# befelix/safe_learning

Measured on AMD Instinct MI355X. Metric: grid-cell Lyapunov checks/sec + ms/safe_set-update, 4D 128^4 grid, 1k-pt GP, higher is better.
Workload: dtype f64

## Files before the change

### include/sl_hip.h

```cpp
#ifndef SL_HIP_H
#define SL_HIP_H

#include <stdint.h>

#ifdef __cplusplus
extern "C" {
#endif

#define SL_API __attribute__((visibility("default")))

#define SL_OK               0
#define SL_ERR_INVALID     (-1)
#define SL_ERR_HIP         (-2)
#define SL_ERR_UNSUPPORTED (-3)
#define SL_ERR_NOMEM       (-4)

#define SL_MAX_STATE_DIM   6
#define SL_MAX_ACTION_DIM  2
#define SL_MAX_INPUT_DIM   8
#define SL_MAX_GP_HEADS    6
#define SL_MAX_NN_LAYERS   4
#define SL_MAX_SIMPLICES   32

typedef struct sl_ctx sl_ctx;
// ... 89 lines not shown
SL_API int  sl_version(void);
SL_API int  sl_ctx_create(int device, void* hip_stream, sl_ctx** out);
SL_API int  sl_ctx_destroy(sl_ctx* ctx);
SL_API const char* sl_last_error(const sl_ctx* ctx);
SL_API int  sl_ctx_synchronize(sl_ctx* ctx);
SL_API const char* sl_last_kernel(const sl_ctx* ctx);
SL_API int  sl_timing_configure(sl_ctx* ctx, int slots);
SL_API int  sl_timing_collect(sl_ctx* ctx, int channel, double* h_ms, int capacity, int* count);

SL_API int  sl_model_set(sl_ctx* ctx, const sl_model_desc* h_model);
SL_API int  sl_policy_touch(sl_ctx* ctx);

SL_API int  sl_gp_set_head(sl_ctx* ctx, int head, int n, int p, int dout, int col0,
                    const double* h_X, const double* h_Linv, const double* h_alpha,
                    double variance, const double* h_lengthscales);
#define SL_KERNEL_RBF 0
#define SL_KERNEL_MATERN32 1
#define SL_KERNEL_LINEAR 2
#define SL_KERNEL_MAX_FACTORS 8
typedef struct sl_gp_kernel_factor {
    int32_t kind, product;
    double  variance[SL_MAX_INPUT_DIM];
    double  inv_lengthscales[SL_MAX_INPUT_DIM];
} sl_gp_kernel_factor;
typedef struct sl_gp_kernel {
    int32_t nfactors, reserved;
    sl_gp_kernel_factor factor[SL_KERNEL_MAX_FACTORS];
} sl_gp_kernel;
SL_API int  sl_gp_set_head_kernel(sl_ctx* ctx, int head, int n, int p, int dout, int col0,
                    const double* h_X, const double* h_Linv, const double* h_alpha,
                    const sl_gp_kernel* h_kernel);
SL_API int  sl_gp_append_point(sl_ctx* ctx, int head, const double* h_x, const double* h_linv_row,
                        const double* h_alpha_new);
SL_API int  sl_gp_configure(sl_ctx* ctx, int nheads, double beta);
SL_API int  sl_gp4_early_configure(sl_ctx* ctx, int enable);
SL_API int  sl_gp4_workgroups_configure(sl_ctx* ctx, int workgroups);
SL_API int  sl_gp4_segment_configure(sl_ctx* ctx, int tiles);

SL_API int  sl_tri_set(sl_ctx* ctx, int slot, const sl_grid_desc* h_grid, int nsimplex,
                const int32_t* h_simplices, const double* h_hyperplanes,
                const double* h_discrete_points, int project, int ncols, const double* d_table);
SL_API int  sl_tri_set_table(sl_ctx* ctx, int slot, const double* d_table);

SL_API int  sl_network_set(sl_ctx* ctx, int nlayers, const int32_t* h_dims ,
                    const int32_t* h_activations, const double* h_kernels);

SL_API int  sl_policy_network_set(sl_ctx* ctx, int nlayers, const int32_t* h_dims,
                           const int32_t* h_activations, const double* h_kernels,
                           const double* h_biases, const int32_t* h_has_bias, double output_scale);

SL_API int  sl_values(sl_ctx* ctx, int64_t lo, int64_t hi, double* d_values);

SL_API int  sl_lyap_sweep(sl_ctx* ctx, int64_t lo, int64_t hi, const uint64_t* d_init_bits,
                   const double* d_values, uint64_t* d_neg_bits, sl_sweep_result* d_result,
                   double* d_dbg);


SL_API int  sl_values_implicit(sl_ctx* ctx, int* out);

SL_API int  sl_fold_results(sl_ctx* ctx, const sl_sweep_result* d_records, int count,
                     sl_sweep_result* d_out);

SL_API int  sl_lyap_finalize_dev(sl_ctx* ctx, int64_t lo, int64_t hi, const double* d_values,
                          const uint64_t* d_init_bits, const uint64_t* d_prev_bits,
                          const sl_sweep_result* d_folded, const sl_key* d_keep,
                          uint64_t* d_safe_bits, sl_sweep_result* d_result);
// ... 150 lines not shown
```

### safe_learning_amd/_hip.py

```python

import ctypes as C
import os

import numpy as np

HERE = os.path.dirname(os.path.abspath(__file__))
LIB_PATH = os.environ.get("SL_LIB_PATH") or os.path.join(HERE, "libslhip.so")

MAX_STATE_DIM = 6
MAX_ACTION_DIM = 2
MAX_INPUT_DIM = 8
MAX_GP_HEADS = 6
MAX_NN_LAYERS = 4
MAX_SIMPLICES = 32

OK, ERR_INVALID, ERR_HIP, ERR_UNSUPPORTED, ERR_NOMEM = 0, -1, -2, -3, -4
POLICY_LINEAR, POLICY_CONST, POLICY_TABLE, POLICY_TRI, POLICY_NETWORK = 1, 2, 3, 4, 5
DYN_LINEAR, DYN_PENDULUM, DYN_CARTPOLE, DYN_GP = 1, 2, 3, 4
V_QUADRATIC, V_TRI, V_NETWORK = 1, 2, 3
LIP_CONST, LIP_ABS_LINEAR, LIP_NORM_LINEAR, LIP_ABS_GRAD, LIP_NORM_GRAD = 0, 1, 2, 3, 4
LF_CONST, LF_AFFINE_NORM1 = 0, 1
EVAL_VALUE, EVAL_POLICY, EVAL_DYNAMICS, EVAL_DECREASE, EVAL_LV = 1, 2, 3, 4, 5
NN_LOSS_ABS, NN_LOSS_ROA = 1, 2

# ... 74 lines not shown
                ("jacobi_cycles", C.c_int64), ("residual_inf", C.c_double), ("bound", C.c_double),
                ("kappa", C.c_double), ("converged", C.c_int32), ("reserved", C.c_int32)]


SOLVE_GMRES, SOLVE_JACOBI = 0, 1


RESULT_WORDS = 8
R_FAIL_V, R_FAIL_I, R_LAST_V, R_LAST_I, R_MAX_V, R_MAX_I, R_BELOW, R_SAFE = range(8)
SORT_COUNT_WORDS = 256 * 2048
ADAPTIVE_ROW_WORDS = 6
SELECT_WORDS = 8
S_PREFIX, S_REMAINING, S_KEY_V, S_KEY_I, S_RANK, S_NONE = range(6)

_vp, _i64, _int, _dbl = C.c_void_p, C.c_int64, C.c_int, C.c_double
_int32_p = C.POINTER(C.c_int32)

SIGNATURES = {
    "sl_version": (_int, ()),
    "sl_ctx_create": (_int, (_int, _vp, C.POINTER(_vp))),
    "sl_ctx_destroy": (_int, (_vp,)),
    "sl_last_error": (C.c_char_p, (_vp,)),
    "sl_ctx_synchronize": (_int, (_vp,)),
    "sl_last_kernel": (C.c_char_p, (_vp,)),
    "sl_timing_configure": (_int, (_vp, _int)),
    "sl_timing_collect": (_int, (_vp, _int, c_double_p, _int, C.POINTER(_int))),
    "sl_model_set": (_int, (_vp, C.POINTER(ModelDesc))),
    "sl_policy_touch": (_int, (_vp,)),
    "sl_gp_set_head": (_int, (_vp, _int, _int, _int, _int, _int, c_double_p, c_double_p, c_double_p, _dbl,
                              c_double_p)),
    "sl_gp_set_head_kernel": (_int, (_vp, _int, _int, _int, _int, _int, c_double_p, c_double_p, c_double_p,
                                     C.POINTER(GpKernel))),
    "sl_gp_append_point": (_int, (_vp, _int, c_double_p, c_double_p, c_double_p)),
    "sl_gp_configure": (_int, (_vp, _int, _dbl)),
    "sl_gp4_early_configure": (_int, (_vp, _int)),
    "sl_gp4_workgroups_configure": (_int, (_vp, _int)),
    "sl_gp4_segment_configure": (_int, (_vp, _int)),
    "sl_tri_set": (_int, (_vp, _int, C.POINTER(GridDesc), _int, _int32_p, c_double_p, c_double_p, _int, _int,
                          _vp)),
    "sl_tri_set_table": (_int, (_vp, _int, _vp)),
    "sl_network_set": (_int, (_vp, _int, _int32_p, _int32_p, c_double_p)),
    "sl_policy_network_set": (_int, (_vp, _int, _int32_p, _int32_p, c_double_p, c_double_p, _int32_p, _dbl)),
    "sl_values": (_int, (_vp, _i64, _i64, _vp)),
    "sl_lyap_sweep": (_int, (_vp, _i64, _i64, _vp, _vp, _vp, _vp, _vp)),
    "sl_values_implicit": (_int, (_vp, C.POINTER(_int))),
    "sl_fold_results": (_int, (_vp, _vp, _int, _vp)),
    "sl_lyap_finalize_dev": (_int, (_vp, _i64, _i64, _vp, _vp, _vp, _vp, _vp, _vp, _vp)),
    "sl_refinement_carry": (_int, (_vp, _i64, _i64, _vp, _vp, _vp, _vp, _vp, _vp)),
    "sl_select_begin": (_int, (_vp, _vp, _i64, _i64, _vp, _i64)),
    "sl_select_hist": (_int, (_vp, _i64, _i64, _vp, _int, _int, _vp, _vp)),
    "sl_select_digit": (_int, (_vp, _int, _int, _vp, _vp)),
    "sl_sort_pairs": (_int, (_vp, _i64, _vp, _vp, _vp, _vp, _vp)),
    "sl_partition_by_digit": (_int, (_vp, _i64, _vp, _vp, _vp, _vp)),
    "sl_gather_rows": (_int, (_vp, _i64, _int, _vp, _vp, _vp)),
    "sl_adaptive_pack": (_int, (_vp, _i64, _i64, _vp, _vp, _int, _vp, _vp, _vp, _vp)),
    "sl_adaptive_dest": (_int, (_vp, _i64, _vp, _vp, _int, _vp)),
    "sl_adaptive_sort_keys": (_int, (_vp, _i64, _vp, _vp, _vp)),
    "sl_adaptive_analyse": (_int, (_vp, _i64, _i64, _i64, _vp, _vp, _dbl, _dbl, _i64, _vp, _vp)),
    "sl_adaptive_apply": (_int, (_vp, _i64, _i64, _i64, _vp, _vp, _vp, _dbl, _dbl, _i64, _vp)),
    "sl_adaptive_scatter": (_int, (_vp, _i64, _i64, _i64, _vp, _vp, _vp, _vp, _vp)),
    "sl_index_to_state": (_int, (_vp, _i64, _vp, _vp)),
    "sl_perturb_pairs": (_int, (_vp, _i64, _int, _int, _vp, _vp, _int, _vp, _vp, _vp)),
    "sl_rows_sort_key": (_int, (_vp, _i64, _int, _int, _vp, _vp, _vp)),
    "sl_rows_duplicate_flags": (_int, (_vp, _i64, _int, _vp, _vp, _vp)),
    "sl_sample_bounds": (_int, (_vp, _i64, _int, _int, _vp, _vp, _vp, _dbl, _vp, _vp)),
    "sl_state_membership": (_int, (_vp, _i64, _vp, _vp, _vp)),
# ... 145 lines not shown
        alpha, pA = _as_c(alpha)
        ls, pls = _as_c(lengthscales)
        n, p = X.shape
        self.lib.sl_gp_set_head(self.handle, head, n, p, alpha.shape[1], col0, pX, pL, pA, float(variance),
                                pls)

    def gp_set_head_kernel(self, head, X, Linv, alpha, col0, factors):
        X, pX = _as_c(X)
        Linv, pL = _as_c(Linv)
        alpha, pA = _as_c(alpha)
        n, p = X.shape
        if len(factors) > KERNEL_MAX_FACTORS:
            raise ValueError("kernel with %d leaf factors (engine limit %d)" % (len(factors), KERNEL_MAX_FACTORS))
        spec = GpKernel()
        spec.nfactors = len(factors)
        for f, (kind, product, variance, inv_ls) in enumerate(factors):
            spec.factor[f].kind, spec.factor[f].product = int(kind), int(product)
            for q in range(p):
                spec.factor[f].variance[q] = float(variance[q])
                spec.factor[f].inv_lengthscales[q] = float(inv_ls[q])
        self.lib.sl_gp_set_head_kernel(self.handle, head, n, p, alpha.shape[1], col0, pX, pL, pA,
                                       C.byref(spec))

    def gp_append_point(self, head, x, linv_row, alpha_new):
        x, px = _as_c(x)
        row, pr = _as_c(linv_row)
        a, pa = _as_c(alpha_new)
        rc = self.lib.sl_gp_append_point(self.handle, head, px, pr, pa)
        if rc == ERR_UNSUPPORTED:
            return False
        self.check(rc, "sl_gp_append_point")
        return True

    def gp_inputs(self, head, n, p):
        out = np.empty((p, n), dtype=np.float64)
        self.lib.sl_debug_gp_inputs(self.handle, head, out.ctypes.data_as(c_double_p))
        return out

    def gp_configure(self, nheads, beta):
        self.lib.sl_gp_configure(self.handle, nheads, float(beta))

    def tri_set(self, slot, grid_desc, simplices, hyperplanes, discrete_points, project, ncols,
                table):
        simplices = np.ascontiguousarray(simplices, dtype=np.int32)
        hyper, ph = _as_c(hyperplanes)
        pts, pp = _as_c(np.concatenate(discrete_points))
        self._keepalive[slot] = table
        self.lib.sl_tri_set(self.handle, slot, C.byref(grid_desc), len(simplices),
                            simplices.ctypes.data_as(C.POINTER(C.c_int32)), ph, pp, int(bool(project)),
                            ncols, _ptr(table))

    def tri_set_table(self, slot, table):
        self._keepalive[slot] = table
        self.lib.sl_tri_set_table(self.handle, slot, _ptr(table))

    def network_set(self, dims, activations, kernels):
        dims = np.ascontiguousarray(dims, dtype=np.int32)
        acts = np.ascontiguousarray(activations, dtype=np.int32)
        flat, pk = _as_c(np.concatenate([np.asarray(k, dtype=np.float64).ravel() for k in kernels]))
        self.lib.sl_network_set(self.handle, len(acts), dims.ctypes.data_as(C.POINTER(C.c_int32)),
                                acts.ctypes.data_as(C.POINTER(C.c_int32)), pk)

    def policy_network_set(self, dims, activations, kernels, biases, output_scale):
        dims = np.ascontiguousarray(dims, dtype=np.int32)
        acts = np.ascontiguousarray(activations, dtype=np.int32)
        flat, pk = _as_c(np.concatenate([np.asarray(k, dtype=np.float64).ravel() for k in kernels]))
# ... 278 lines not shown
```

### safe_learning_amd/csrc/sl_gp.hip

```cpp
#include "sl_common.h"

typedef double sl_d4 __attribute__((ext_vector_type(4)));
typedef double sl_d2 __attribute__((ext_vector_type(2)));

#define SL_GP_SLABS_PER_CHUNK 16
#ifndef SL_GP_STAGGER
#define SL_GP_STAGGER 1
#endif
#ifndef SL_GP_GEN_UNROLL
#define SL_GP_GEN_UNROLL 1
#endif
#define SL_GP_DOUT_MAX SL_MAX_STATE_DIM

static constexpr int kCfgW[2] = {4, 8};
static constexpr int kCfgR[2] = {1, 4};
static constexpr int kCfgCB[2] = {1, 4};

static inline int cfg_panel_rows(int cfg) { return 16 * kCfgR[cfg != 0] * kCfgW[cfg != 0]; }

template <int W, int R, int CB, bool GENERAL, int DT, int MT, bool XSG = false>
__global__ __launch_bounds__(W * 64) void k_gp_sweep(
    const SlDevModel M, const SlGpDev gp, SlAux aux_arg, int64_t lo, int64_t hi, int64_t ntiles,
    const uint64_t* __restrict__ init_bits, const double* __restrict__ values,
    uint64_t* __restrict__ neg_bits, sl_key* __restrict__ partials, double* __restrict__ dbg,
    int xs_doubles, int alpha_doubles, const double* __restrict__ points, int nb_arg) {
    __shared__ SlTriLds<GENERAL> tri_lds;
    const SlAux aux = sl_stage_aux<GENERAL>(tri_lds, aux_arg);
    constexpr int C = 16 * CB;
    constexpr int RP = 16 * R * W;
    constexpr int RB = R * W;
    constexpr int FRAGS = SL_GP_SLABS_PER_CHUNK * CB / W;
    constexpr int KXBUF = SL_GP_SLABS_PER_CHUNK * CB * 64;
    static_assert(W % CB == 0, "W must be a multiple of CB");
// ... 283 lines not shown
    }
    __syncthreads();
    sl_block_reduce_key<true>(best_v, best_i, sv, si);
    if (tid == 0) { partials[blockIdx.x].vbits = best_v; partials[blockIdx.x].index = best_i; }
}

static int choose_cfg(const sl_ctx* ctx, int n) {
    if (ctx->env.gp_cfg >= 0) return ctx->env.gp_cfg;
    if (n <= 256) return 0;
    return 2;
}

static int gp_set_head(sl_ctx* ctx, int head, int n, int p, int dout, int col0, const double* h_X,
                       const double* h_Linv, const double* h_alpha, double variance,
                       const double* h_lengthscales, const sl_gp_kernel* h_kernel) {
    if (!ctx || !h_X || !h_Linv || !h_alpha || !h_lengthscales)
        return sl_fail(ctx, SL_ERR_INVALID, "sl_gp_set_head: NULL argument");
    if (head < 0 || head >= SL_MAX_GP_HEADS)
        return sl_fail(ctx, SL_ERR_INVALID, "sl_gp_set_head: head %d outside [0,%d)", head,
                       SL_MAX_GP_HEADS);
    if (n < 1 || p < 1 || p > SL_MAX_INPUT_DIM || dout < 1 || col0 < 0 ||
        col0 + dout > SL_MAX_STATE_DIM)
        return sl_fail(ctx, SL_ERR_INVALID, "sl_gp_set_head: bad sizes n=%d p=%d dout=%d col0=%d",
                       n, p, dout, col0);
    if (!(variance > 0.0)) return sl_fail(ctx, SL_ERR_INVALID, "sl_gp_set_head: variance <= 0");
    for (int q = 0; q < p; ++q)
        if (!(h_lengthscales[q] > 0.0))
            return sl_fail(ctx, SL_ERR_INVALID, "sl_gp_set_head: lengthscale <= 0");
    const int cfg = choose_cfg(ctx, n);
    const int rp = cfg_panel_rows(cfg);
    const int n_pad = ((n + rp - 1) / rp) * rp;
    const int nslab2 = n_pad / 8;

    std::vector<double> xs((size_t)p * n_pad, 0.0), alphap((size_t)n_pad * dout, 0.0);
    std::vector<double> mpack((size_t)n_pad * n_pad, 0.0);
    for (int j = 0; j < n; ++j)
        for (int q = 0; q < p; ++q) xs[(size_t)q * n_pad + j] = h_X[(size_t)j * p + q] / h_lengthscales[q];
    for (int i = 0; i < n; ++i) {
        for (int dd = 0; dd < dout; ++dd) {
            const double ai = h_alpha[(size_t)i * dout + dd];
            if (ai == 0.0) continue;
            for (int j = 0; j <= i; ++j) alphap[(size_t)j * dout + dd] += h_Linv[(size_t)i * n + j] * ai;
        }
    }
    for (int I = 0; I < n_pad / 16; ++I) {
        for (int S2 = 0; S2 < nslab2; ++S2) {
            if (8 * S2 > 16 * I + 15) continue;
            for (int l = 0; l < 64; ++l) {
                const int row = 16 * I + (l & 15);
                for (int e = 0; e < 2; ++e) {
                    const int col = 4 * (2 * S2 + e) + (l >> 4);
                    double v = 0.0;
                    if (row < n && col <= row) v = h_Linv[(size_t)row * n + col];
                    mpack[(((size_t)I * nslab2 + S2) * 64 + l) * 2 + e] = v;
                }
            }
        }
    }
    SL_HIP_CHECK(ctx, hipSetDevice(ctx->device));
    SL_HIP_CHECK(ctx, hipStreamSynchronize(ctx->stream));
    ++ctx->dynamics_token;
    SlGpHeadHost& hh = ctx->gp_heads[head];
    if (hh.d_xs) (void)hipFree(hh.d_xs);
    if (hh.d_mpack) (void)hipFree(hh.d_mpack);
    if (hh.d_alpha) (void)hipFree(hh.d_alpha);
    if (hh.d_kernel) (void)hipFree(hh.d_kernel);
    hh.d_xs = hh.d_mpack = hh.d_alpha = nullptr;
    hh.d_kernel = nullptr;
    if (h_kernel) {
        SL_HIP_CHECK(ctx, hipMalloc(&hh.d_kernel, sizeof(sl_gp_kernel)));
        SL_HIP_CHECK(ctx, hipMemcpy(hh.d_kernel, h_kernel, sizeof(sl_gp_kernel), hipMemcpyHostToDevice));
        hh.h_kernel = *h_kernel;
    }
    SL_HIP_CHECK(ctx, hipMalloc(&hh.d_xs, xs.size() * sizeof(double)));
    SL_HIP_CHECK(ctx, hipMalloc(&hh.d_mpack, mpack.size() * sizeof(double)));
    SL_HIP_CHECK(ctx, hipMalloc(&hh.d_alpha, alphap.size() * sizeof(double)));
// ... 67 lines not shown
    }
}

extern "C" int sl_gp_append_point(sl_ctx* ctx, int head, const double* h_x, const double* h_linv_row,
                                  const double* h_alpha_new) {
    if (!ctx || !h_x || !h_linv_row || !h_alpha_new)
        return sl_fail(ctx, SL_ERR_INVALID, "sl_gp_append_point: NULL argument");
    if (head < 0 || head >= SL_MAX_GP_HEADS || !ctx->gp_heads[head].set)
        return sl_fail(ctx, SL_ERR_INVALID, "sl_gp_append_point: head %d not set", head);
    SlGpHeadHost& hh = ctx->gp_heads[head];
    SlGpHeadDev& dv = ctx->h_gp.head[head];
    const int n = hh.n;
    if (n + 1 > hh.n_pad)
        return sl_fail(ctx, SL_ERR_UNSUPPORTED, "sl_gp_append_point: capacity %d of head %d is "
                                                "exhausted (upload the head again)", hh.n_pad, head);
    ++ctx->dynamics_token;
    SL_HIP_CHECK(ctx, hipSetDevice(ctx->device));
    SL_HIP_CHECK(ctx, hipStreamSynchronize(ctx->stream));
    const size_t need = sizeof(double) * (size_t)(n + 1 + hh.p + hh.dout);
    SL_HIP_CHECK(ctx, sl_grow(ctx, &ctx->d_scratch, &ctx->scratch_bytes, need));
    std::vector<double> stage((size_t)(n + 1 + hh.p + hh.dout));
    for (int c = 0; c <= n; ++c) stage[c] = h_linv_row[c];
    for (int q = 0; q < hh.p; ++q) stage[n + 1 + q] = h_x[q] / hh.lengthscales[q];
    for (int dd = 0; dd < hh.dout; ++dd) stage[n + 1 + hh.p + dd] = h_alpha_new[dd];
    double* d_stage = reinterpret_cast<double*>(ctx->d_scratch);
    SL_HIP_CHECK(ctx, hipMemcpy(d_stage, stage.data(), need, hipMemcpyHostToDevice));
    hipLaunchKernelGGL(k_gp_append, dim3((n + hh.p + 256) / 256), dim3(256), 0, ctx->stream, d_stage, n,
                       hh.n_pad, dv.nslab2, hh.p, hh.dout, d_stage + n + 1, d_stage + n + 1 + hh.p,
                       hh.d_mpack, hh.d_alpha, hh.d_xs);
    SL_HIP_CHECK(ctx, hipGetLastError());
    SL_HIP_CHECK(ctx, hipStreamSynchronize(ctx->stream));
    hh.n = n + 1;
    dv.n = n + 1;
    SL_HIP_CHECK(ctx, hipMemcpy(ctx->d_gp, &ctx->h_gp, sizeof(SlGpDev), hipMemcpyHostToDevice));
    return SL_OK;
}

extern "C" int sl_debug_gp_inputs(sl_ctx* ctx, int head, double* h_xs) {
    if (!ctx || !h_xs) return sl_fail(ctx, SL_ERR_INVALID, "sl_debug_gp_inputs: NULL argument");
    if (head < 0 || head >= SL_MAX_GP_HEADS || !ctx->gp_heads[head].set)
        return sl_fail(ctx, SL_ERR_INVALID, "sl_debug_gp_inputs: head %d not set", head);
    const SlGpHeadHost& hh = ctx->gp_heads[head];
    SL_HIP_CHECK(ctx, hipSetDevice(ctx->device));
    SL_HIP_CHECK(ctx, hipStreamSynchronize(ctx->stream));
    for (int q = 0; q < hh.p; ++q)
        SL_HIP_CHECK(ctx, hipMemcpy(h_xs + (size_t)q * hh.n, hh.d_xs + (size_t)q * hh.n_pad,
                                    sizeof(double) * hh.n, hipMemcpyDeviceToHost));
    return SL_OK;
}

extern "C" int sl_gp4_early_configure(sl_ctx* ctx, int enable) {
    if (!ctx) return sl_fail(nullptr, SL_ERR_INVALID, "sl_gp4_early_configure: NULL context");
    ctx->gp4_early = enable != 0;
    return SL_OK;
}

extern "C" int sl_gp_configure(sl_ctx* ctx, int nheads, double beta) {
    if (!ctx) return sl_fail(nullptr, SL_ERR_INVALID, "sl_gp_configure: NULL context");
    if (nheads < 1 || nheads > SL_MAX_GP_HEADS)
        return sl_fail(ctx, SL_ERR_INVALID, "sl_gp_configure: %d heads", nheads);
    int cfg = -1;
    for (int h = 0; h < nheads; ++h) {
        if (!ctx->gp_heads[h].set)
            return sl_fail(ctx, SL_ERR_INVALID, "sl_gp_configure: head %d not set", h);
        if (cfg < 0) cfg = ctx->gp_heads[h].cfg;
        if (cfg != ctx->gp_heads[h].cfg)
            return sl_fail(ctx, SL_ERR_UNSUPPORTED,
// ... 306 lines not shown
```

### safe_learning_amd/csrc/sl_gp4.hip

```cpp
#include "sl_common.h"
#include "sl_gp4_clobbers.h"
#include "sl_gp4_gen.h"
#include "sl_gp4_mean.h"
#include "sl_gp4_queue.h"

#ifdef SL_NO_GP4
bool sl_gp4_supports(const SlDevModel&) { return false; }
int sl_gp4_sweep_launch(sl_ctx* ctx, const SlDevModel&, const SlSweepArgs&, int*) {
    return sl_fail(ctx, SL_ERR_UNSUPPORTED, "k_gp_sweep4 is compiled out of this build");
}
extern "C" int sl_gp4_workgroups_configure(sl_ctx*, int) { return SL_OK; }
extern "C" int sl_gp4_segment_configure(sl_ctx*, int) { return SL_OK; }
#else

namespace gp4 {

#ifndef SL_GP4_R
#define SL_GP4_R 4
#endif
constexpr int R = SL_GP4_R, CB = 4, W = 4;
constexpr int NACC = R * CB * 4;
constexpr int C = 16 * CB;
constexpr int RP = 16 * R * W;
constexpr int RB = R * W;
#ifndef SL_GP4_WRITE_SKEW
#define SL_GP4_WRITE_SKEW 1
#endif
constexpr int KXS2 = CB * 128 + 4;
constexpr int KXBUF = 8 * KXS2;
static_assert(R == 4, "256-row panels (tools/audit_gp4.py is told the same number by the build)");

constexpr int REC_MEAN = 8, REC_SS = REC_MEAN + 16 * SL_D, REC = REC_SS + W * 16;
struct BlockCtl {
    Gp4Queues q;
    int action;
    int pos[GP4Q_SLOTS];
    int open[W];
    int push_stage;
    int src_done;
    int nsrc;
    int from_list;
    unsigned nlist;
};
constexpr int ACT_SOURCE = GP4Q_SOURCE, ACT_DONE = GP4Q_DONE;

struct AFrag { sl_d2 v[R]; };
struct BFrag { sl_d2 v[CB]; };

#define SL_A10(b) "a" #b "0", "a" #b "1", "a" #b "2", "a" #b "3", "a" #b "4", "a" #b "5", "a" #b "6", "a" #b "7", "a" #b "8", "a" #b "9"
#define SL_AGPRS_0_127                                                                             \
    "a0", "a1", "a2", "a3", "a4", "a5", "a6", "a7", "a8", "a9", SL_A10(1), SL_A10(2), SL_A10(3),   \
        SL_A10(4), SL_A10(5), SL_A10(6), SL_A10(7), SL_A10(8), SL_A10(9), SL_A10(10), SL_A10(11),   \
        "a120", "a121", "a122", "a123", "a124", "a125", "a126", "a127"
#define SL_ALL_AGPRS SL_AGPRS_0_127

template <int BASE>
__device__ __forceinline__ void acc_zero16() {
    asm volatile(
        "v_accvgpr_write_b32 a%c0, 0\n\tv_accvgpr_write_b32 a%c1, 0\n\tv_accvgpr_write_b32 a%c2, 0\n\t"
        "v_accvgpr_write_b32 a%c3, 0\n\tv_accvgpr_write_b32 a%c4, 0\n\tv_accvgpr_write_b32 a%c5, 0\n\t"
        "v_accvgpr_write_b32 a%c6, 0\n\tv_accvgpr_write_b32 a%c7, 0\n\tv_accvgpr_write_b32 a%c8, 0\n\t"
        "v_accvgpr_write_b32 a%c9, 0\n\tv_accvgpr_write_b32 a%c10, 0\n\tv_accvgpr_write_b32 a%c11, 0\n\t"
        "v_accvgpr_write_b32 a%c12, 0\n\tv_accvgpr_write_b32 a%c13, 0\n\tv_accvgpr_write_b32 a%c14, 0\n\t"
// ... 515 lines not shown
                const double* kxr = kx_l + buf * KXBUF + wave * 128 + own;
                sl_d2 kx[8];
                load_own_kx<KXS2>(kx, kxr);
                mean_mfma(kx, mi, macc);
            };
            auto produce = [&](int ch, int buf, int first_new, bool keep) {
                const bool with_mean = ch >= first_new && !(skip & 2);
                MeanIn mi;
                if (with_mean) load_alpha(mi, rs_alpha, lk, low, dout, ch);
                if (!(skip & 1)) generate(ch, buf, first_new, keep);
                if (with_mean) {
                    __builtin_amdgcn_fence(__ATOMIC_RELEASE, "wavefront");
                    __builtin_amdgcn_wave_barrier();
                    mean_run(buf, mi);
                }
            };

            const int npanels = (hd.n + RP - 1) / RP;
            constexpr int CPP = RP / 64;
            const int nchunks_head = npanels * CPP;
            auto decide_block = [&](int done) -> bool {
                const bool last = done == npanels;
                const int64_t idx = blk0 + lcol;
                const bool valid = lk == 0 && idx < hi;
                const int cl = 16 * wave + lcol;
                CellBounds b{false, false, 0.0};
                if (valid) {
                    double var = variance;
                    if (done > 0) {
                        double sumsq = 0.0;
                        for (int k = 0; k < PSS; ++k) sumsq += part_ss[k * C + cl];
                        var = variance - sumsq;
                    }
                    b = cell_bounds(M, nd, aux, gp.beta, idx, lo, points, values, cell_mean + cl * SL_D, var);
                }
                const bool neg_hi = b.neg_hi, open = b.open;
                const double v_x = b.v_x;
                const bool all = last || __ballot(open) == 0ull;
                if (all) {
                    const unsigned word = (unsigned)(__ballot(neg_hi) & 0xffffull);
                    const int64_t b16 = (blk0 - lo) >> 4;
                    unsigned init = 0u;
                    if (init_bits) init = reinterpret_cast<const unsigned short*>(init_bits)[b16];
                    if (lane == 0) reinterpret_cast<unsigned short*>(neg_bits)[b16] = (unsigned short)word;
                    const bool okc = neg_hi || ((init >> lcol) & 1u);
                    if (valid && !okc) sl_key_min(best_v, best_i, sl_vbits(v_x), idx);
#ifdef SL_DIAG
                    if (lane == 0 && !last && done < 4) atomicAdd(&sl_gp4_stage_count[done], 1ull);
#endif
                }
                return all;
            };
            if (early && stage == ACT_SOURCE) {
                for (int ch = 0; ch < nchunks_head; ++ch) produce(ch, ch & 1, 0, false);
                if (lk < dout)
                    cell_mean[(16 * wave + 4 * blk + low) * SL_D + hd.col0 + lk] = mean_sum(macc);
            }
#ifdef SL_DIAG
            if (early && stage >= 0 && stage < 4 && tid == 0) atomicAdd(&sl_gp4_stage_count[4 + stage], 1ull);
#endif
            for (int pan = early ? (stage >= 0 ? stage : npanels) : (decided ? npanels : 0);
                 pan < (early ? stage + 1 : npanels); ++pan) {
                acc_zero_all();
                int rowoff[R];
                int nzd[R];
#pragma unroll
                for (int r = 0; r < R; ++r) {
// ... 301 lines not shown
```

### safe_learning_amd/csrc/sl_gp4_gen.h

```cpp
#pragma once
#include "sl_common.h"

typedef double sl_d2 __attribute__((ext_vector_type(2)));
typedef unsigned sl_u4 __attribute__((ext_vector_type(4)));

namespace gp4 {

constexpr int RUNS = 4;
constexpr int RUNC = SL_P + 2;

__device__ __forceinline__ void exp_pair(double x1, double x2, double& e1, double& e2) {
    x1 = x1 < -800.0 ? -800.0 : x1;
    x2 = x2 < -800.0 ? -800.0 : x2;
    const double k1 = rint(x1 * 1.4426950408889634), k2 = rint(x2 * 1.4426950408889634);
    double r1 = fma(k1, -6.93147180369123816490e-01, x1), r2 = fma(k2, -6.93147180369123816490e-01, x2);
    r1 = fma(k1, -1.90821492927058770002e-10, r1);
    r2 = fma(k2, -1.90821492927058770002e-10, r2);
    double q1 = 1.6059043836821613e-10, q2 = 1.6059043836821613e-10;
#define SL_EXP_STEP(C) q1 = fma(q1, r1, C); q2 = fma(q2, r2, C)
    SL_EXP_STEP(2.08767569878681e-09);
    SL_EXP_STEP(2.505210838544172e-08);
    SL_EXP_STEP(2.755731922398589e-07);
    SL_EXP_STEP(2.7557319223985893e-06);
    SL_EXP_STEP(2.48015873015873e-05);
// ... 66 lines not shown
            rs_alpha, voff, (64 * ch + 8 * s2) * dout * 8, 0));
        mi.a1[s2] = __builtin_bit_cast(double, __builtin_amdgcn_raw_buffer_load_b64(
            rs_alpha, voff, (64 * ch + 8 * s2 + 4) * dout * 8, 0));
    }
}
template <int KXS2>
__device__ __forceinline__ void load_own_kx(sl_d2 (&kx)[8], const double* kxr) {
#pragma unroll
    for (int s2 = 0; s2 < 8; ++s2) kx[s2] = *reinterpret_cast<const sl_d2*>(kxr + s2 * KXS2);
}
__device__ __forceinline__ void mean_mfma(const sl_d2 (&kx)[8], const MeanIn& mi, double (&macc)[4]) {
#pragma unroll
    for (int h = 0; h < 2; ++h)
        asm volatile("s_nop 3\n\t"
                     "v_mfma_f64_4x4x4_4b_f64 %0, %4, %5, %0\n\t"
                     "v_mfma_f64_4x4x4_4b_f64 %1, %6, %7, %1\n\t"
                     "v_mfma_f64_4x4x4_4b_f64 %2, %8, %9, %2\n\t"
                     "v_mfma_f64_4x4x4_4b_f64 %3, %10, %11, %3\n\t"
                     "v_mfma_f64_4x4x4_4b_f64 %0, %12, %13, %0\n\t"
                     "v_mfma_f64_4x4x4_4b_f64 %1, %14, %15, %1\n\t"
                     "v_mfma_f64_4x4x4_4b_f64 %2, %16, %17, %2\n\t"
                     "v_mfma_f64_4x4x4_4b_f64 %3, %18, %19, %3"
                     : "+v"(macc[0]), "+v"(macc[1]), "+v"(macc[2]), "+v"(macc[3])
                     : "v"(mi.a0[4 * h]), "v"(kx[4 * h].x), "v"(mi.a1[4 * h]), "v"(kx[4 * h].y),
                       "v"(mi.a0[4 * h + 1]), "v"(kx[4 * h + 1].x), "v"(mi.a1[4 * h + 1]), "v"(kx[4 * h + 1].y),
                       "v"(mi.a0[4 * h + 2]), "v"(kx[4 * h + 2].x), "v"(mi.a1[4 * h + 2]), "v"(kx[4 * h + 2].y),
                       "v"(mi.a0[4 * h + 3]), "v"(kx[4 * h + 3].x), "v"(mi.a1[4 * h + 3]), "v"(kx[4 * h + 3].y));
    asm volatile("s_nop 15\n\ts_nop 7" : "+v"(macc[0]), "+v"(macc[1]), "+v"(macc[2]), "+v"(macc[3]));
}
__device__ __forceinline__ double mean_sum(const double (&macc)[4]) {
    return (macc[0] + macc[1]) + (macc[2] + macc[3]);
}

struct CellBounds { bool neg_hi, open; double v_x; };
__device__ __forceinline__ CellBounds cell_bounds(const SlDevModel& M, const SlDims& nd, const SlAux& aux, double beta,
                                                  int64_t idx, int64_t lo, const double* points, const double* values,
                                                  const double* mean_row, double var) {
    const int d = nd.d, p = nd.p;
    double x[SL_P], u[SL_M], prior[SL_D], mean[SL_D], err0[SL_D], err1[SL_D];
    sl_cell_state(M, d, idx, points, x);
    sl_policy_any<false>(M, nd, aux.tri, idx, x, u);
    sl_append_action(nd, u, x);
    sl_rows_dot<SL_D, SL_P>(M.m.dynamics.matrix, d, p, x, prior);
    const double e = beta * sqrt(var);
#pragma unroll
    for (int k = 0; k < SL_D; ++k) {
        if (k < d) {
            mean[k] = mean_row[k] + prior[k];
            err0[k] = 0.0;
            err1[k] = e;
        }
    }
    const SlCellCheck c0 = sl_cell_check<SL_FAST>(M, d, aux, x, mean, err0);
    const SlCellCheck c1 = sl_cell_check<SL_FAST>(M, d, aux, x, mean, err1);
    CellBounds b;
    b.neg_hi = c1.negative;
    b.open = c0.negative != c1.negative || !(fabs(c0.decrease) < INFINITY) || !(fabs(c1.decrease) < INFINITY);
    b.v_x = values ? values[idx - lo] : c1.v_x;
    return b;
}

}
```

### safe_learning_amd/csrc/sl_gp4_mean.hip

```cpp
#include "sl_common.h"
#include "sl_gp4_gen.h"
#include "sl_gp4_mean.h"
#include "sl_gp4_queue.h"

#ifndef SL_NO_GP4

namespace gp4m {

using gp4::RUNC;
using gp4::RUNS;
using gp4::uniform;

constexpr int W = 4;
constexpr int WG_PER_CU = 4;
constexpr int KXS2 = 128 + 4;
constexpr int KXBUF = 8 * KXS2;
constexpr int SLICE = KXBUF + 16 * SL_P + RUNS * RUNC;
static_assert(16 * SL_D <= KXBUF, "the block's means reuse the chunk buffer");
static_assert(W * SLICE * sizeof(double) <= 40 * 1024, "four workgroups of k_gp_mean_blocks per CU");

}

#ifdef SL_DIAG
static __device__ unsigned long long sl_gp4_mean_decided;
// ... 167 lines not shown
                        for (int c = c0; c < c1; ++c) {
                            kxw[2 * ((c + wswz) & 15)] = e;
                            e *= rho;
                            rho *= qr;
                        }
                    }
                } else {
                    gp4::direct_run(kxw, wswz, xv, cin, 0, variance, p);
                }
            };
            for (int ch = 0; ch < nchunks_head; ++ch) {
                const bool with_mean = !(skip & 2);
                gp4::MeanIn mi;
                if (with_mean) gp4::load_alpha(mi, rs_alpha, lk, low, dout, ch);
                if (!(skip & 1)) generate(ch);
                if (with_mean) {
                    __builtin_amdgcn_fence(__ATOMIC_RELEASE, "wavefront");
                    __builtin_amdgcn_wave_barrier();
                    sl_d2 kx[8];
                    gp4::load_own_kx<KXS2>(kx, kx_l + own);
                    gp4::mean_mfma(kx, mi, macc);
                }
            }
            __builtin_amdgcn_fence(__ATOMIC_RELEASE, "wavefront");
            __builtin_amdgcn_wave_barrier();
            if (lk < dout) cell_mean[(4 * blk + low) * SL_D + hd.col0 + lk] = gp4::mean_sum(macc);
            __builtin_amdgcn_fence(__ATOMIC_RELEASE, "wavefront");
            __builtin_amdgcn_wave_barrier();

            const int64_t idx = blk0 + lcol;
            const bool valid = lk == 0 && idx < hi;
            gp4::CellBounds b{false, false, 0.0};
            if (valid)
                b = gp4::cell_bounds(M, nd, aux, gp.beta, idx, lo, points, values, cell_mean + lcol * SL_D, variance);
            const bool neg_hi = b.neg_hi, open = b.open;
            const double v_x = b.v_x;
            if (__ballot(open) == 0ull) {
                const unsigned word = (unsigned)(__ballot(neg_hi) & 0xffffull);
                const int64_t b16 = (blk0 - lo) >> 4;
                unsigned init = 0u;
                if (init_bits) init = reinterpret_cast<const unsigned short*>(init_bits)[b16];
                if (lane == 0) reinterpret_cast<unsigned short*>(neg_bits)[b16] = (unsigned short)word;
                const bool okc = neg_hi || ((init >> lcol) & 1u);
                if (valid && !okc) sl_key_min(best_v, best_i, sl_vbits(v_x), idx);
#ifdef SL_DIAG
                if (lane == 0) atomicAdd(&sl_gp4_mean_decided, 1ull);
#endif
            } else {
                unsigned at = 0u;
                if (lane == 0) at = atomicAdd(list_count, 1u);
                at = (unsigned)__builtin_amdgcn_readfirstlane((int)at);
                if (at < list_cap) {
                    if (lane == 0) list_cell[at] = blk0;
                    double* rec = list_mean + (size_t)at * 16 * d;
                    for (int i = lane; i < 16 * d; i += 64) rec[i] = cell_mean[(i / d) * SL_D + i % d];
                }
            }
            __builtin_amdgcn_fence(__ATOMIC_RELEASE, "wavefront");
            __builtin_amdgcn_wave_barrier();
        }
    }
    sl_wave_reduce_key<true>(best_v, best_i);
    if (lane == 0) {
        sl_key* out = partials + blockIdx.x * W + wave;
        if (fold) sl_key_min(best_v, best_i, out->vbits, out->index);
        out->vbits = best_v;
        out->index = best_i;
// ... 56 lines not shown
```

### safe_learning_amd/csrc/sl_model.h

```cpp
#pragma once

#include <stdint.h>
#include <math.h>
#include <string.h>
#include "sl_hip.h"

#if defined(__HIPCC__)
#define SL_HD __host__ __device__ __forceinline__
#else
#define SL_HD inline
#endif

#define SL_D SL_MAX_STATE_DIM
#define SL_M SL_MAX_ACTION_DIM
#define SL_P SL_MAX_INPUT_DIM

#define SL_TRI_CODES   64
#define SL_TRI_MAXCAND 12
struct SlTri {
    sl_grid_desc grid;
    int32_t nsimplex, project, ncols, set;
    int32_t simplices[SL_MAX_SIMPLICES][SL_D + 1];
    double  hyper[SL_MAX_SIMPLICES][SL_D][SL_D];
    double  hyper_c[SL_MAX_SIMPLICES][SL_D];
// ... 827 lines not shown
SL_HD double sl_tanh(double x) {
#if defined(__HIP_DEVICE_COMPILE__)
    double y = -2.0 * fabs(x);
    y = y < -80.0 ? -80.0 : y;
    const double k = rint(y * 1.4426950408889634);
    double r = fma(k, -6.93147180369123816490e-01, y);
    r = fma(k, -1.90821492927058770002e-10, r);
    double q = 1.6059043836821613e-10;
    q = fma(q, r, 2.08767569878681e-09);
    q = fma(q, r, 2.505210838544172e-08);
    q = fma(q, r, 2.755731922398589e-07);
    q = fma(q, r, 2.7557319223985893e-06);
    q = fma(q, r, 2.48015873015873e-05);
    q = fma(q, r, 1.984126984126984e-04);
    q = fma(q, r, 1.3888888888888889e-03);
    q = fma(q, r, 8.333333333333333e-03);
    q = fma(q, r, 4.1666666666666664e-02);
    q = fma(q, r, 1.6666666666666666e-01);
    q = fma(q, r, 0.5);
    q = fma(q, r, 1.0);
    const double e = ldexp(fma(q, r, 1.0), (int)k);
    const double em1 = (k == 0.0) ? q * r : e - 1.0;
    const double t = (0.0 - em1) / (2.0 + em1);
    return copysign(t, x);
#else
    return tanh(x);
#endif
}
SL_HD double sl_act(int a, double x) { return a == 1 ? sl_tanh(x) : (a == 2 ? (x > 0.0 ? x : 0.0) : x); }
SL_HD double sl_dact(int a, double pre, double post) {
    return a == 1 ? (1.0 - post * post) : (a == 2 ? (pre > 0.0 ? 1.0 : 0.0) : 1.0);
}

struct SlGpHeadDev {
    int32_t n, n_pad, p, dout, col0, nslab2, reserved0, reserved1;
    double  variance;
    double  inv_ls[SL_P];
    const double* xs;
    const double* mpack;
    const double* alpha;
    const sl_gp_kernel* kernel;
};

SL_HD double sl_kernel_eval(const sl_gp_kernel& ks, int p, const double* a, const double* b) {
    double total = 0.0, prod = 1.0;
    int cur = 0;
    for (int f = 0; f < ks.nfactors; ++f) {
        const sl_gp_kernel_factor& fac = ks.factor[f];
        if (fac.product != cur) {
            total += prod;
            prod = 1.0;
            cur = fac.product;
        }
        double v = 0.0;
        if (fac.kind == SL_KERNEL_LINEAR) {
#pragma unroll
            for (int q = 0; q < SL_P; ++q)
                if (q < p) v = fma(a[q] * fac.variance[q], b[q], v);
        } else {
            double r2 = 0.0;
#pragma unroll
            for (int q = 0; q < SL_P; ++q) {
                if (q < p) {
                    const double dq = (a[q] - b[q]) * fac.inv_lengthscales[q];
                    r2 = fma(dq, dq, r2);
                }
// ... 370 lines not shown
```

Measured before the change: 272.1 million.

## Add certified GP variance lower bound to close cells earlier in staged gp4

```diff
diff --git a/include/sl_hip.h b/include/sl_hip.h
--- a/include/sl_hip.h
+++ b/include/sl_hip.h
@@ -145,6 +145,7 @@
                     const sl_gp_kernel* h_kernel);
 SL_API int  sl_gp_append_point(sl_ctx* ctx, int head, const double* h_x, const double* h_linv_row,
                         const double* h_alpha_new);
+SL_API int  sl_gp_variance_floor(sl_ctx* ctx, int head, double* out, int n);
 SL_API int  sl_gp_configure(sl_ctx* ctx, int nheads, double beta);
 SL_API int  sl_gp4_early_configure(sl_ctx* ctx, int enable);
 SL_API int  sl_gp4_workgroups_configure(sl_ctx* ctx, int workgroups);
diff --git a/safe_learning_amd/_hip.py b/safe_learning_amd/_hip.py
--- a/safe_learning_amd/_hip.py
+++ b/safe_learning_amd/_hip.py
@@ -130,6 +130,7 @@
     "sl_gp_set_head_kernel": (_int, (_vp, _int, _int, _int, _int, _int, c_double_p, c_double_p, c_double_p,
                                      C.POINTER(GpKernel))),
     "sl_gp_append_point": (_int, (_vp, _int, c_double_p, c_double_p, c_double_p)),
+    "sl_gp_variance_floor": (_int, (_vp, _int, c_double_p, _int)),
     "sl_gp_configure": (_int, (_vp, _int, _dbl)),
     "sl_gp4_early_configure": (_int, (_vp, _int)),
     "sl_gp4_workgroups_configure": (_int, (_vp, _int)),
@@ -341,6 +342,11 @@
         self.check(rc, "sl_gp_append_point")
         return True
 
+    def gp_variance_floor(self, head, stages):
+        out = np.zeros(stages, dtype=np.float64)
+        self.lib.sl_gp_variance_floor(self.handle, head, out.ctypes.data_as(c_double_p), stages)
+        return out
+
     def gp_inputs(self, head, n, p):
         out = np.empty((p, n), dtype=np.float64)
         self.lib.sl_debug_gp_inputs(self.handle, head, out.ctypes.data_as(c_double_p))
diff --git a/safe_learning_amd/csrc/sl_gp.hip b/safe_learning_amd/csrc/sl_gp.hip
--- a/safe_learning_amd/csrc/sl_gp.hip
+++ b/safe_learning_amd/csrc/sl_gp.hip
@@ -1,4 +1,5 @@
 #include "sl_common.h"
+#include "sl_gp_floor.h"
 
 typedef double sl_d4 __attribute__((ext_vector_type(4)));
 typedef double sl_d2 __attribute__((ext_vector_type(2)));
@@ -348,7 +349,7 @@
     const int n_pad = ((n + rp - 1) / rp) * rp;
     const int nslab2 = n_pad / 8;
 
-    std::vector<double> xs((size_t)p * n_pad, 0.0), alphap((size_t)n_pad * dout, 0.0);
+    std::vector<double> xs((size_t)p * n_pad, 0.0), alphap((size_t)n_pad * dout + SL_GP_FLOOR_WORDS, 0.0);
     std::vector<double> mpack((size_t)n_pad * n_pad, 0.0);
     for (int j = 0; j < n; ++j)
         for (int q = 0; q < p; ++q) xs[(size_t)q * n_pad + j] = h_X[(size_t)j * p + q] / h_lengthscales[q];
@@ -358,6 +359,14 @@
             if (ai == 0.0) continue;
             for (int j = 0; j <= i; ++j) alphap[(size_t)j * dout + dd] += h_Linv[(size_t)i * n + j] * ai;
         }
+    }
+    const int floor_stages = (n + SL_GP_FLOOR_RP - 1) / SL_GP_FLOOR_RP;
+    if (!h_kernel && ctx->gp4_early && ctx->env.gp_cfg < 0 && n_pad % SL_GP_FLOOR_RP == 0 &&
+        floor_stages <= SL_GP_FLOOR_STAGES && n <= SL_GP_FLOOR_MAX_N) {
+        double floor_c[SL_GP_FLOOR_STAGES] = {};
+        gpfloor::variance_floor(h_Linv, n, SL_GP_FLOOR_RP, floor_stages, variance, floor_c);
+        alphap[(size_t)n_pad * dout] = 2.0 * 64.0 * (double)n * 0x1p-53 * variance;
+        for (int s = 0; s < floor_stages; ++s) alphap[(size_t)n_pad * dout + 1 + s] = floor_c[s];
     }
     for (int I = 0; I < n_pad / 16; ++I) {
         for (int S2 = 0; S2 < nslab2; ++S2) {
@@ -491,7 +500,23 @@
     SL_HIP_CHECK(ctx, hipStreamSynchronize(ctx->stream));
     hh.n = n + 1;
     dv.n = n + 1;
+    SL_HIP_CHECK(ctx, hipMemset(hh.d_alpha + (size_t)hh.n_pad * hh.dout, 0, SL_GP_FLOOR_WORDS * sizeof(double)));
     SL_HIP_CHECK(ctx, hipMemcpy(ctx->d_gp, &ctx->h_gp, sizeof(SlGpDev), hipMemcpyHostToDevice));
+    return SL_OK;
+}
+
+extern "C" int sl_gp_variance_floor(sl_ctx* ctx, int head, double* out, int n) {
+    if (!ctx || !out) return sl_fail(ctx, SL_ERR_INVALID, "sl_gp_variance_floor: NULL argument");
+    if (head < 0 || head >= SL_MAX_GP_HEADS || !ctx->gp_heads[head].set)
+        return sl_fail(ctx, SL_ERR_INVALID, "sl_gp_variance_floor: head %d not set", head);
+    if (n < 0 || n > SL_GP_FLOOR_STAGES)
+        return sl_fail(ctx, SL_ERR_INVALID, "sl_gp_variance_floor: %d constants outside [0,%d]", n, SL_GP_FLOOR_STAGES);
+    const SlGpHeadHost& hh = ctx->gp_heads[head];
+    SL_HIP_CHECK(ctx, hipSetDevice(ctx->device));
+    SL_HIP_CHECK(ctx, hipStreamSynchronize(ctx->stream));
+    if (n > 0)
+        SL_HIP_CHECK(ctx, hipMemcpy(out, hh.d_alpha + (size_t)hh.n_pad * hh.dout + 1, sizeof(double) * n,
+                                    hipMemcpyDeviceToHost));
     return SL_OK;
 }
 
diff --git a/safe_learning_amd/csrc/sl_gp4.hip b/safe_learning_amd/csrc/sl_gp4.hip
--- a/safe_learning_amd/csrc/sl_gp4.hip
+++ b/safe_learning_amd/csrc/sl_gp4.hip
@@ -29,6 +29,8 @@
 constexpr int KXS2 = CB * 128 + 4;
 constexpr int KXBUF = 8 * KXS2;
 static_assert(R == 4, "256-row panels (tools/audit_gp4.py is told the same number by the build)");
+static_assert(RP == SL_GP_FLOOR_RP && GP4Q_STAGES == SL_GP_FLOOR_STAGES,
+              "sl_gp_set_head computes the variance floor for these panel boundaries");
 
 constexpr int REC_MEAN = 8, REC_SS = REC_MEAN + 16 * SL_D, REC = REC_SS + W * 16;
 struct BlockCtl {
@@ -610,7 +612,10 @@
                         for (int k = 0; k < PSS; ++k) sumsq += part_ss[k * C + cl];
                         var = variance - sumsq;
                     }
-                    b = cell_bounds(M, nd, aux, gp.beta, idx, lo, points, values, cell_mean + cl * SL_D, var);
+                    const double* fw = floor_words(hd);
+                    const double floor_c = last ? 0.0 : fw[1 + done], floor_2d = last ? 0.0 : fw[0];
+                    b = cell_bounds<true>(M, nd, aux, gp.beta, idx, lo, points, values, cell_mean + cl * SL_D, var,
+                                          floor_c, floor_2d);
                 }
                 const bool neg_hi = b.neg_hi, open = b.open;
                 const double v_x = b.v_x;
diff --git a/safe_learning_amd/csrc/sl_gp4_gen.h b/safe_learning_amd/csrc/sl_gp4_gen.h
--- a/safe_learning_amd/csrc/sl_gp4_gen.h
+++ b/safe_learning_amd/csrc/sl_gp4_gen.h
@@ -122,10 +122,15 @@
     return (macc[0] + macc[1]) + (macc[2] + macc[3]);
 }
 
+__device__ __forceinline__ const double* floor_words(const SlGpHeadDev& hd) {
+    return hd.alpha + (size_t)hd.n_pad * hd.dout;
+}
+
 struct CellBounds { bool neg_hi, open; double v_x; };
+template <bool FLOOR>
 __device__ __forceinline__ CellBounds cell_bounds(const SlDevModel& M, const SlDims& nd, const SlAux& aux, double beta,
                                                   int64_t idx, int64_t lo, const double* points, const double* values,
-                                                  const double* mean_row, double var) {
+                                                  const double* mean_row, double var, double floor_c, double floor_2d) {
     const int d = nd.d, p = nd.p;
     double x[SL_P], u[SL_M], prior[SL_D], mean[SL_D], err0[SL_D], err1[SL_D];
     sl_cell_state(M, d, idx, points, x);
@@ -133,11 +138,12 @@
     sl_append_action(nd, u, x);
     sl_rows_dot<SL_D, SL_P>(M.m.dynamics.matrix, d, p, x, prior);
     const double e = beta * sqrt(var);
+    const double e_lo = FLOOR ? beta * sqrt(fmax(floor_c * var - floor_2d, 0.0)) : 0.0;
 #pragma unroll
     for (int k = 0; k < SL_D; ++k) {
         if (k < d) {
             mean[k] = mean_row[k] + prior[k];
-            err0[k] = 0.0;
+            err0[k] = e_lo;
             err1[k] = e;
         }
     }
diff --git a/safe_learning_amd/csrc/sl_gp4_mean.hip b/safe_learning_amd/csrc/sl_gp4_mean.hip
--- a/safe_learning_amd/csrc/sl_gp4_mean.hip
+++ b/safe_learning_amd/csrc/sl_gp4_mean.hip
@@ -223,7 +223,8 @@
             const bool valid = lk == 0 && idx < hi;
             gp4::CellBounds b{false, false, 0.0};
             if (valid)
-                b = gp4::cell_bounds(M, nd, aux, gp.beta, idx, lo, points, values, cell_mean + lcol * SL_D, variance);
+                b = gp4::cell_bounds<false>(M, nd, aux, gp.beta, idx, lo, points, values, cell_mean + lcol * SL_D, variance,
+                                            0.0, 0.0);
             const bool neg_hi = b.neg_hi, open = b.open;
             const double v_x = b.v_x;
             if (__ballot(open) == 0ull) {
diff --git a/safe_learning_amd/csrc/sl_gp_floor.h b/safe_learning_amd/csrc/sl_gp_floor.h
--- /dev/null
+++ b/safe_learning_amd/csrc/sl_gp_floor.h
@@ -0,0 +1,118 @@
+#pragma once
+
+#include <cmath>
+#include <limits>
+#include <vector>
+
+namespace gpfloor {
+
+constexpr int FLOOR_ITERATIONS = 300;
+constexpr int FLOOR_RETRIES = 8;
+constexpr double FLOOR_MARGIN = 1e-3;
+
+template <typename T>
+inline T dot4(const T* a, const T* b, int n) {
+    T s0 = 0, s1 = 0, s2 = 0, s3 = 0;
+    int j = 0;
+    for (; j + 4 <= n; j += 4) {
+        s0 += a[j] * b[j];
+        s1 += a[j + 1] * b[j + 1];
+        s2 += a[j + 2] * b[j + 2];
+        s3 += a[j + 3] * b[j + 3];
+    }
+    for (; j < n; ++j) s0 += a[j] * b[j];
+    return (s0 + s1) + (s2 + s3);
+}
+
+inline bool cholesky_runs(std::vector<long double>& a, int k) {
+    for (int i = 0; i < k; ++i) {
+        long double* ai = &a[(size_t)i * k];
+        for (int j = 0; j < i; ++j) {
+            const long double* aj = &a[(size_t)j * k];
+            ai[j] = (ai[j] - dot4(ai, aj, j)) / aj[j];
+        }
+        const long double piv = ai[i] - dot4(ai, ai, i);
+        if (!(piv > 0.0L) || !(piv < (long double)INFINITY)) return false;
+        ai[i] = std::sqrt(piv);
+    }
+    return true;
+}
+
+inline double lambda_min_certified(const double* Linv, int n, int m) {
+    const int k = n - m;
+    if (k < 1) return 0.0;
+    auto B = [&](int r) { return Linv + (size_t)(m + r) * n + m; };
+    for (int r = 0; r < k; ++r)
+        if (!(B(r)[r] > 0.0)) return 0.0;
+    std::vector<double> x(k), y(k), w(k);
+    unsigned state = 12345u;
+    for (int i = 0; i < k; ++i) {
+        state = state * 1664525u + 1013904223u;
+        x[i] = 0.5 + (double)(state >> 8) / (double)(1u << 24);
+    }
+    double theta = 0.0;
+    for (int it = 0; it < FLOOR_ITERATIONS; ++it) {
+        double nx = std::sqrt(dot4(x.data(), x.data(), k));
+        if (!(nx > 0.0) || !(nx < INFINITY)) return 0.0;
+        for (int i = 0; i < k; ++i) w[i] = x[i] = x[i] / nx;
+        for (int i = k - 1; i >= 0; --i) {
+            const double* bi = B(i);
+            const double zi = w[i] / bi[i];
+            w[i] = zi;
+            for (int j = 0; j < i; ++j) w[j] -= bi[j] * zi;
+        }
+        for (int i = 0; i < k; ++i) {
+            const double* bi = B(i);
+            y[i] = (w[i] - dot4(bi, y.data(), i)) / bi[i];
+        }
+        const double yx = dot4(y.data(), x.data(), k), yy = dot4(y.data(), y.data(), k);
+        if (!(yx > 0.0) || !(yy > 0.0) || !(yy < INFINITY)) return 0.0;
+        const double rq = yx / yy;
+        const bool settled = it > 0 && std::fabs(rq - theta) <= 1e-7 * rq;
+        theta = rq;
+        x.swap(y);
+        if (settled) break;
+    }
+    std::vector<long double> P((size_t)k * k, 0.0L), A((size_t)k * k), row(k);
+    for (int r = 0; r < k; ++r) {
+        const double* br = B(r);
+        for (int j = 0; j <= r; ++j) row[j] = br[j];
+        for (int i = 0; i <= r; ++i) {
+            const long double bri = row[i];
+            long double* pi = &P[(size_t)i * k];
+            for (int j = 0; j <= i; ++j) pi[j] += bri * row[j];
+        }
+    }
+    long double pnorm = 0.0L;
+    for (int i = 0; i < k; ++i) {
+        long double sum = 0.0L;
+        for (int j = 0; j < k; ++j) sum += std::fabs(j <= i ? P[(size_t)i * k + j] : P[(size_t)j * k + i]);
+        pnorm = sum > pnorm ? sum : pnorm;
+    }
+    if (!(pnorm < (long double)INFINITY)) return 0.0;
+    const double round = (double)(64.0L * k * std::numeric_limits<long double>::epsilon() * pnorm);
+    double step = FLOOR_MARGIN;
+    for (int attempt = 0; attempt < FLOOR_RETRIES; ++attempt, step *= 2.0) {
+        const double t = theta * (1.0 - step);
+        A = P;
+        for (int i = 0; i < k; ++i) A[(size_t)i * k + i] -= t;
+        if (cholesky_runs(A, k)) return t > round ? t - round : 0.0;
+    }
+    return 0.0;
+}
+
+inline void variance_floor(const double* h_Linv, int n, int rp, int stages, double variance, double* floor_c) {
+    for (int s = 0; s < stages; ++s) floor_c[s] = 0.0;
+    if (n < 1 || rp < 1 || !(variance > 0.0) || !(variance < INFINITY)) return;
+    for (int i = 0; i < n; ++i)
+        for (int j = 0; j <= i; ++j)
+            if (!(std::fabs(h_Linv[(size_t)i * n + j]) < INFINITY)) return;
+    const double noise = 1.0 / (h_Linv[0] * h_Linv[0]) - variance;
+    if (!(noise > 0.0) || !(noise < INFINITY)) return;
+    for (int s = 0; s < stages && s * rp < n; ++s) {
+        const double c = noise * (1.0 - FLOOR_MARGIN) * lambda_min_certified(h_Linv, n, s * rp);
+        floor_c[s] = (c > 0.0 && c < 1.0) ? c : 0.0;
+    }
+}
+
+}
diff --git a/safe_learning_amd/csrc/sl_model.h b/safe_learning_amd/csrc/sl_model.h
--- a/safe_learning_amd/csrc/sl_model.h
+++ b/safe_learning_amd/csrc/sl_model.h
@@ -883,6 +883,10 @@
     return a == 1 ? (1.0 - post * post) : (a == 2 ? (pre > 0.0 ? 1.0 : 0.0) : 1.0);
 }
 
+#define SL_GP_FLOOR_STAGES 32
+#define SL_GP_FLOOR_WORDS (1 + SL_GP_FLOOR_STAGES)
+#define SL_GP_FLOOR_RP 256
+#define SL_GP_FLOOR_MAX_N 2048
 struct SlGpHeadDev {
     int32_t n, n_pad, p, dout, col0, nslab2, reserved0, reserved1;
     double  variance;
```

Measured after the change: 296.4 million (median of 6 runs). 8.9% higher.
